# microsoft/SpeechT5

Hardware: AMD Instinct MI355X
Metric: audio-sec/s fwd+bwd SpeechT5-Base (higher is better)
Workload: dtype bf16

## Files before the change

### include/speecht5_hip.h

```cpp
#ifndef SPEECHT5_HIP_H
#define SPEECHT5_HIP_H
#include <stdint.h>
#ifdef __cplusplus
extern "C" {
#endif

#define ST5_F32 0
#define ST5_BF16 1

#define ST5_ACT_NONE 0
#define ST5_ACT_GELU 1
#define ST5_ACT_RELU 2
#define ST5_ACT_TANH 3
#define ST5_ACT_LRELU_01 4
#define ST5_ACT_LRELU_001 5

#define ST5_GEMM_A_KSTRIDED 1
#define ST5_GEMM_B_KSTRIDED 2
#define ST5_GEMM_OUT_F32 4
#define ST5_GEMM_DACT 8
#define ST5_GEMM_DEFERRABLE 16

typedef struct st5_operand {
  const void* ptr;
// ... 251 lines not shown
                     const int64_t* target_lengths, int32_t T, int32_t B, int32_t V, int32_t max_target_len, int32_t blank,
                     int32_t zero_infinity, const float* nll, const float* grad_out, const void* ws, float* grad, void* stream);
int64_t st5_guided_attn_ws_bytes(void);
int st5_guided_attn_fwd(const float* att, const int64_t* ilens, const int64_t* olens, int32_t B, int32_t H, int32_t To, int32_t Ti,
                        float sigma, float alpha, float* out2, void* ws, void* stream);
int st5_guided_attn_bwd(const int64_t* ilens, const int64_t* olens, int32_t B, int32_t H, int32_t To, int32_t Ti, float sigma,
                        const float* out2, const float* grad_out, float* datt, void* stream);
int64_t st5_vq_ws_bytes(void);
int32_t st5_vq_vpad(void);
int st5_vq_fwd(const float* logits, const float* gumbel, const float* vars, const void* enc, const float* mix_w, float tau, const float* tau_dev,
               int32_t training, void* out, int32_t* idx, float* avg, float* perp2, void* ws, int32_t N, int32_t G, int32_t V, int32_t Dg,
               int32_t T, int dtype, void* stream);
int st5_vq_bwd(const float* logits, const float* gumbel, const float* dsel, int32_t dsel_ld, const float* avg, const float* g_prob_perp,
               const void* dout, const float* mix_w, float tau, const float* tau_dev, int32_t training, float* dlogits, void* denc, int32_t N,
               int32_t G, int32_t V, int32_t Dg, int32_t T, int dtype, void* stream);
int st5_norm_rows(const void* x, float* y, float* inv, int64_t rows, int32_t cols, int dtype, void* stream);
int st5_norm_rows_bwd(const float* y, const float* inv, const float* dy, void* dx, int64_t rows, int32_t cols, int32_t accumulate, int dtype,
                      void* stream);
int st5_canon_rows(const float* e, int32_t* canon, int32_t V, int32_t D, void* stream);
int st5_nce_logits(const float* sim, const int32_t* target, const int32_t* canon, float* logits, int64_t S, int32_t V, float temp, void* stream);
int st5_nce_logits_bwd(const float* dlogits, const int32_t* target, const int32_t* canon, float* dsim, int32_t dsim_ld, int64_t S, int32_t V,
                       float temp, void* stream);
int st5_layernorm_set_max_blocks(int n);
int st5_ctc_initial_state(const float* x, int32_t T, int32_t V, int32_t blank, float* r, void* stream);
int st5_ctc_prefix_score(const float* x, int32_t T, int32_t V, int32_t blank, int32_t eos, const float* r_prev, const int64_t* last,
                         int32_t out_len, const int64_t* cs, int32_t nh, int32_t nc, float* log_psi, float* r_new, void* stream);
int st5_ctc_initial_state_rows(const float* x, const int32_t* lens, int32_t S, int32_t Tmax, int32_t V, int32_t blank, float* r, void* stream);
int st5_ctc_prefix_score_rows(const float* x, const int32_t* lens, const int32_t* sent, int32_t S, int32_t Tmax, int32_t V, int32_t blank,
                              int32_t eos, const float* r_prev, const int64_t* last, int32_t out_len, const int64_t* cs, int32_t nh,
                              int32_t nc, float* log_psi, float* r_new, void* stream);
int st5_ctc_select_rows(const int32_t* lens, const int32_t* sent, int32_t S, int32_t Tmax, const int64_t* cs, int32_t nh, int32_t nc,
                        const float* log_psi, const float* r_new, const int64_t* parent, const int64_t* token, int32_t n, float* state,
                        float* prev_psi, uint8_t* known, int32_t* sent_out, void* stream);
int64_t st5_lm_decode_attn_ws_bytes(int32_t rows, int32_t t, int32_t H, int32_t head_dim);
int st5_lm_decode_attn(const void* q, int64_t q_ld, const void* kv, int32_t rows_cap, int32_t Tmax, const int32_t* anc, int64_t anc_ld,
                       int32_t rows, int32_t t, int32_t H, int32_t head_dim, void* ctx, int64_t ctx_ld, float* ws, int dtype, void* stream);
int st5_lm_reorder(const int32_t* anc, int64_t anc_ld, const int64_t* order, int32_t rows_old, int32_t rows_new, int32_t t, int32_t Tmax,
                   int32_t* anc_new, int64_t new_ld, void* stream);
int st5_lm_fuse_logprobs(float* lprobs, int64_t lp_ld, const void* logits, int64_t lg_ld, int32_t rows, int32_t V_lm, float lm_weight,
                         int dtype, void* stream);
int64_t st5_decode_cross_attn_ws_bytes(int32_t B, int32_t S, int32_t H, int32_t head_dim);
int st5_decode_cross_attn(const void* q, int64_t q_ld, const void* kv, int64_t kv_ld, int64_t k_off, const uint8_t* kpm, int32_t B,
                          int32_t S, int32_t H, int32_t head_dim, void* ctx, int64_t ctx_ld, float* probs, int64_t p_row, int64_t p_head,
                          float* ws, int dtype, void* stream);
int st5_tts_step_tail(const float* y, int64_t y_ld, int32_t B, int32_t r, int32_t odim, const int32_t* minlen, const int32_t* maxlen,
                      int32_t* done, int32_t* steps, int32_t idx, int32_t cap, float threshold, float* mel, float* probs, void* next,
// ... 59 lines not shown
```

### speecht5_amd/csrc/norm.hip

```cpp
#include "common.h"
#include "../../include/speecht5_hip.h"

namespace {

constexpr int MAXCH = 8;

template <typename T, int NCH>
__device__ __forceinline__ void load_row(const T* row, int cols, int lane, bool vec, float (&v)[NCH][8]) {
#pragma unroll
  for (int i = 0; i < NCH; ++i) {
    const int c = i * 512 + lane * 8;
    if (c < cols) {
      if (vec) load8f<T>(row + c, v[i]);
      else {
#pragma unroll
        for (int e = 0; e < 8; ++e) v[i][e] = (c + e < cols) ? Elem<T>::to_f(row[c + e]) : 0.f;
      }
    } else {
#pragma unroll
      for (int e = 0; e < 8; ++e) v[i][e] = 0.f;
    }
  }
}
template <typename T, int NCH>
// ... 335 lines not shown
        const long long r2 = r1 + stride;
        if (r2 < rows) load_set(A, r2);
        finish_set(B, r1);
        if (r2 >= rows) break;
        row0 = r2;
      }
    }
  }
  if (PG) {
#pragma unroll
    for (int i = 0; i < NV; ++i) {
      const int c = (i * 64 + lane) * 4;
      if (c < cols) {
#pragma unroll
        for (int e = 0; e < 4; ++e) { red[(wave * 2 + 0) * cols + c + e] = dg[i][e]; red[(wave * 2 + 1) * cols + c + e] = db[i][e]; }
      }
    }
    __syncthreads();
    for (int c = threadIdx.x; c < 2 * cols; c += 256)
      part[(long long)blockIdx.x * 2 * cols + c] = red[c] + red[2 * cols + c] + red[4 * cols + c] + red[6 * cols + c];
  }
}

__global__ __launch_bounds__(1024) void ln_bwd_final_kernel(const float* __restrict__ part, float* __restrict__ dgamma,
                                                            float* __restrict__ dbeta, int nblk, int cols) {
  __shared__ float red[16][64];
  const int cl = threadIdx.x & 63, j = threadIdx.x >> 6;
  const int c = blockIdx.x * 64 + cl;
  float s = 0.f;
  if (c < 2 * cols)
    for (int b = j; b < nblk; b += 16) s += part[(long long)b * 2 * cols + c];
  red[j][cl] = s;
  __syncthreads();
  if (j == 0 && c < 2 * cols) {
    s = 0.f;
#pragma unroll
    for (int k = 0; k < 16; ++k) s += red[k][cl];
    if (c < cols) { if (dgamma) dgamma[c] += s; }
    else if (dbeta) dbeta[c - cols] += s;
  }
}

constexpr int LNF_MAX = 48;
struct LnFinalDesc { const float* part; float* dgamma; float* dbeta; int nblk, cols, blk0, pad; };
struct LnFinalArgs { LnFinalDesc d[LNF_MAX]; int n; };
__global__ __launch_bounds__(1024) void ln_bwd_final_multi_kernel(const LnFinalArgs a) {
// ... 29 lines not shown
    for (int i = 0; i < g_nlnstates; ++i)
      if (g_lnstates[i].pending.n != 0) return nullptr;
    if (hipDeviceSynchronize() != hipSuccess) return nullptr;
    g_nlnstates = 0;
  }
  LnDeferState* d = &g_lnstates[g_nlnstates++];
  d->stream = s; d->pending.n = 0; d->blocks = 0; d->arena_used = 0;
  return d;
}
#define g_ln_pending (ls->pending)
#define g_ln_blocks (ls->blocks)
#define g_ln_arena (ls->arena)
#define g_ln_arena_bytes (ls->arena_bytes)
#define g_ln_arena_used (ls->arena_used)
int ln_flush_state(LnDeferState* ls) {
  if (!ls || g_ln_pending.n == 0) return ST5_OK;
  hipLaunchKernelGGL(ln_bwd_final_multi_kernel, dim3((unsigned)g_ln_blocks), dim3(1024), 0, ls->stream, g_ln_pending);
  g_ln_pending.n = 0; g_ln_blocks = 0; g_ln_arena_used = 0;
  HIP_CHECK_LAUNCH();
  return ST5_OK;
}
int ln_flush(hipStream_t s) { return ln_flush_state(ln_state(s, false)); }

int ln_blocks(long long rows) {
  long long n = (rows + 4 * BRPW - 1) / (4 * BRPW);
  if (n < 1) n = 1;
  if (n <= g_ln_max_blocks) return (int)n;
  const long long trips = (n + g_ln_max_blocks - 1) / g_ln_max_blocks;
  return (int)((n + trips - 1) / trips);
}

template <typename T, int MODE>
__global__ __launch_bounds__(256) void colreduce_kernel(const T* __restrict__ x, const T* __restrict__ dy,
                                                        const float* __restrict__ mean,
                                                        const float* __restrict__ rstd, float* __restrict__ part,
                                                        long long rows, int cols, long long ld, const float* __restrict__ gate = nullptr) {
  if (st5_gate_dropped(gate)) return;
  __shared__ float red[8][256 + 8];
  const int tx = threadIdx.x & 31, ty = threadIdx.x >> 5;
  const int c0 = blockIdx.x * 256 + tx * 8;
  const bool vec = (ld % 8) == 0 && c0 + 8 <= cols;
  float acc[8];
#pragma unroll
  for (int e = 0; e < 8; ++e) acc[e] = 0.f;
  if (c0 < cols) {
    for (long long r = (long long)blockIdx.y * 8 + ty; r < rows; r += (long long)gridDim.y * 8) {
// ... 57 lines not shown
  dim3 grid((cols + 255) / 256, ns);
  hipLaunchKernelGGL((colreduce_kernel<T, MODE>), grid, dim3(256), 0, s, (const T*)x, (const T*)dy, mean, rstd, ws,
                     rows, cols, ld, gate);
  hipLaunchKernelGGL(colreduce_final_kernel, dim3((cols + 255) / 256), dim3(256), 0, s, ws, out, ns, cols, scale,
                     accumulate, gate);
  HIP_CHECK_LAUNCH();
  return ST5_OK;
}

}

static int layernorm_fwd(const void* x, const float* gamma, const float* beta, void* y, float* mean,
                         float* rstd, int64_t rows, int32_t cols, float eps, int dtype, void* stream, const float* keep, const void* skip,
                         const float* gate = nullptr) {
  if (!x || !y || !gamma || !beta || rows < 0 || cols <= 0 || cols > MAXCH * 512) return ST5_ERR_ARG;
  if (keep && (!skip || cols % 4 != 0 || cols > 2048)) return ST5_ERR_ARG;
  if (gate && ((skip && !keep) || cols % 4 != 0 || cols > 2048)) return ST5_ERR_ARG;
  if (rows == 0) return ST5_OK;
  hipStream_t s = (hipStream_t)stream;
  dim3 grid((unsigned)((rows + 3) / 4));
  if (dtype != ST5_BF16 && dtype != ST5_F32) return ST5_ERR_ARG;
  if (cols % 4 == 0 && cols <= 2048) {
    dim3 vgrid((unsigned)((rows + 4 * RPW - 1) / (4 * RPW)));
#define LNV(TT, NV_)                                                                                                 \
  hipLaunchKernelGGL((ln_fwd_vec_kernel<TT, NV_>), vgrid, dim3(256), 0, s, (const TT*)x, gamma, beta, (TT*)y, mean, rstd, \
                     (long long)rows, cols, eps, keep, (const TT*)skip, (unsigned char*)nullptr, (unsigned char*)nullptr, gate)
#define LNV_T(TT)                                                                                                     \
  do {                                                                                                                \
    if (cols <= 256) LNV(TT, 1); else if (cols <= 512) LNV(TT, 2); else if (cols <= 768) LNV(TT, 3);                  \
    else if (cols <= 1024) LNV(TT, 4); else if (cols <= 1536) LNV(TT, 6); else LNV(TT, 8);                            \
  } while (0)
    if (dtype == ST5_BF16) LNV_T(bf16_t); else LNV_T(float);
#undef LNV_T
#undef LNV
    HIP_CHECK_LAUNCH();
    return ST5_OK;
  }
#define LNF(TT, NCH)                                                                                              \
  hipLaunchKernelGGL((ln_fwd_kernel<TT, NCH>), grid, dim3(256), 0, s, (const TT*)x, gamma, beta, (TT*)y, mean, rstd, \
                     (long long)rows, cols, eps)
#define LNF_T(TT)                                                                                \
  do {                                                                                           \
    if (cols <= 512) LNF(TT, 1); else if (cols <= 1024) LNF(TT, 2); else if (cols <= 2048) LNF(TT, 4); else LNF(TT, 8); \
  } while (0)
  if (dtype == ST5_BF16) LNF_T(bf16_t); else LNF_T(float);
#undef LNF_T
#undef LNF
  HIP_CHECK_LAUNCH();
  return ST5_OK;
}

extern "C" int st5_layernorm_fwd(const void* x, const float* gamma, const float* beta, void* y, float* mean,
                                 float* rstd, int64_t rows, int32_t cols, float eps, int dtype, void* stream) {
  return layernorm_fwd(x, gamma, beta, y, mean, rstd, rows, cols, eps, dtype, stream, nullptr, nullptr);
}
extern "C" int st5_layernorm_fwd_q8(const void* x, const float* gamma, const float* beta, void* y, float* mean, float* rstd, void* q, uint8_t* sc,
                                    int64_t rows, int32_t cols, float eps, void* stream) {
  if (!x || !y || !gamma || !beta || !q || !sc || rows < 0 || cols <= 0 || cols % 32 || cols > 2048) return ST5_ERR_ARG;
  if (rows == 0) return ST5_OK;
  hipStream_t s = (hipStream_t)stream;
  dim3 vgrid((unsigned)((rows + 4 * RPW - 1) / (4 * RPW)));
#define LNQ(NV_)                                                                                                                       \
  hipLaunchKernelGGL((ln_fwd_vec_kernel<bf16_t, NV_, true>), vgrid, dim3(256), 0, s, (const bf16_t*)x, gamma, beta, (bf16_t*)y, mean, rstd, \
                     (long long)rows, cols, eps, (const float*)nullptr, (const bf16_t*)nullptr, (unsigned char*)q, (unsigned char*)sc)
  if (cols <= 256) LNQ(1); else if (cols <= 512) LNQ(2); else if (cols <= 768) LNQ(3);
  else if (cols <= 1024) LNQ(4); else if (cols <= 1536) LNQ(6); else LNQ(8);
#undef LNQ
  HIP_CHECK_LAUNCH();
  return ST5_OK;
}
extern "C" int st5_layernorm_gelu_fwd(const void* x, const float* gamma, const float* beta, void* y, float* mean, float* rstd,
                                      int64_t rows, int32_t cols, float eps, int dtype, void* stream) {
  if (!x || !y || !gamma || !beta || rows < 0 || cols <= 0 || cols % 4 || cols > 512) return ST5_ERR_ARG;
  if (dtype != ST5_BF16 && dtype != ST5_F32) return ST5_ERR_ARG;
  if (rows == 0) return ST5_OK;
  hipStream_t s = (hipStream_t)stream;
  dim3 vgrid((unsigned)((rows + 4 * RPW - 1) / (4 * RPW)));
#define LNA(TT, NV_)                                                                                                                      \
  hipLaunchKernelGGL((ln_fwd_vec_kernel<TT, NV_, false, true>), vgrid, dim3(256), 0, s, (const TT*)x, gamma, beta, (TT*)y, mean, rstd,    \
                     (long long)rows, cols, eps, (const float*)nullptr, (const TT*)nullptr, (unsigned char*)nullptr, (unsigned char*)nullptr)
  if (dtype == ST5_BF16) { if (cols <= 256) LNA(bf16_t, 1); else LNA(bf16_t, 2); }
  else { if (cols <= 256) LNA(float, 1); else LNA(float, 2); }
#undef LNA
  HIP_CHECK_LAUNCH();
  return ST5_OK;
}
extern "C" int st5_layernorm_gelu_bwd(const void* dy, const void* x, const float* gamma, const float* beta, const float* mean, const float* rstd,
                                      void* dx, float* dgamma, float* dbeta, void* ws, int64_t rows, int32_t cols, int dtype, void* stream) {
  if (!dy || !x || !gamma || !beta || !mean || !rstd || !dx || rows < 0 || cols <= 0 || cols % 4 || cols > 512) return ST5_ERR_ARG;
  if ((dgamma || dbeta) && !ws) return ST5_ERR_ARG;
  if (dtype != ST5_BF16 && dtype != ST5_F32) return ST5_ERR_ARG;
  if (rows == 0) return ST5_OK;
  hipStream_t s = (hipStream_t)stream;
  const int nb = ln_blocks(rows);
  const bool pg = dgamma || dbeta;
  const size_t shm = pg ? (size_t)8 * cols * sizeof(float) : 0;
#define LBA(TT, NV_)                                                                                                                       \
  do {                                                                                                                                     \
    if (pg) hipLaunchKernelGGL((ln_bwd_vec_kernel<TT, NV_, true, true>), dim3(nb), dim3(256), shm, s, (const TT*)dy, (const TT*)x, gamma,  \
                               mean, rstd, (TT*)dx, (float*)ws, (long long)rows, cols, (TT*)nullptr, 0.f, 0ull, (const float*)nullptr, beta); \
    else hipLaunchKernelGGL((ln_bwd_vec_kernel<TT, NV_, false, true>), dim3(nb), dim3(256), 0, s, (const TT*)dy, (const TT*)x, gamma,      \
                            mean, rstd, (TT*)dx, (float*)ws, (long long)rows, cols, (TT*)nullptr, 0.f, 0ull, (const float*)nullptr, beta); \
  } while (0)
  if (dtype == ST5_BF16) { if (cols <= 256) LBA(bf16_t, 1); else LBA(bf16_t, 2); }
  else { if (cols <= 256) LBA(float, 1); else LBA(float, 2); }
#undef LBA
  if (pg) hipLaunchKernelGGL(ln_bwd_final_kernel, dim3((2 * cols + 63) / 64), dim3(1024), 0, s, (const float*)ws, dgamma, dbeta, nb, cols);
  HIP_CHECK_LAUNCH();
  return ST5_OK;
}
extern "C" int st5_layernorm_gated_fwd(const void* x, const float* gamma, const float* beta, void* y, float* mean, float* rstd,
                                       int64_t rows, int32_t cols, float eps, const float* keep, const void* skip, int dtype, void* stream) {
  if (!keep || !skip) return ST5_ERR_ARG;
  return layernorm_fwd(x, gamma, beta, y, mean, rstd, rows, cols, eps, dtype, stream, keep, skip);
}
extern "C" int st5_layernorm_fwd_gate(const void* x, const float* gamma, const float* beta, void* y, float* mean, float* rstd, int64_t rows,
                                      int32_t cols, float eps, const float* keep, const void* skip, const float* gate, int dtype,
                                      void* stream) {
  if ((keep == nullptr) != (skip == nullptr)) return ST5_ERR_ARG;
  return layernorm_fwd(x, gamma, beta, y, mean, rstd, rows, cols, eps, dtype, stream, keep, skip, gate);
}

extern "C" int64_t st5_layernorm_bwd_ws_bytes(int64_t rows, int32_t cols) {
  const int64_t a = (int64_t)nsplit_for(rows) * cols * sizeof(float);
  const int64_t b = (int64_t)ln_blocks(rows) * 2 * cols * sizeof(float);
  return a > b ? a : b;
}

static int layernorm_bwd(const void* dy, const void* x, const float* gamma, const float* mean,
// ... 20 lines not shown
      for (int j = 0; j < g_ln_pending.n; ++j)
        if ((dgamma && g_ln_pending.d[j].dgamma == dgamma) || (dbeta && g_ln_pending.d[j].dbeta == dbeta)) {
          const int rc = ln_flush(s); if (rc) return rc; break;
        }
      const size_t need = ((size_t)nb * 2 * cols * sizeof(float) + 255) & ~(size_t)255;
      if (g_ln_pending.n == LNF_MAX || g_ln_arena_used + need > g_ln_arena_bytes) {
        const int rc = ln_flush(s); if (rc) return rc;
        if (need > g_ln_arena_bytes) {
          if (g_ln_arena) (void)hipFree(g_ln_arena);
          size_t want = size_t(128) << 20;
          while (want < need * 4) want *= 2;
          if (st5_dev_malloc(&g_ln_arena, want) != hipSuccess) { g_ln_arena = nullptr; g_ln_arena_bytes = 0; return ST5_ERR_LAUNCH; }
          g_ln_arena_bytes = want;
        }
      }
      ws = reinterpret_cast<char*>(g_ln_arena) + g_ln_arena_used;
      g_ln_arena_used += need;
      LnFinalDesc& d = g_ln_pending.d[g_ln_pending.n++];
      d.part = reinterpret_cast<const float*>(ws); d.dgamma = dgamma; d.dbeta = dbeta; d.nblk = nb; d.cols = cols;
      d.blk0 = g_ln_blocks; d.pad = 0;
      g_ln_blocks += (2 * cols + 63) / 64;
      deferred = true;
    }
#define LBV(TT, NV_)                                                                                                    \
  do {                                                                                                                  \
    if (pg) hipLaunchKernelGGL((ln_bwd_vec_kernel<TT, NV_, true>), dim3(nb), dim3(256), shm, s, (const TT*)dy, (const TT*)x, gamma, \
                               mean, rstd, (TT*)dx, (float*)ws, (long long)rows, cols, (TT*)dx_dropped, drop_p,          \
                               (unsigned long long)drop_seed, keep, (const float*)nullptr, (const TT*)addend, gate);    \
    else hipLaunchKernelGGL((ln_bwd_vec_kernel<TT, NV_, false>), dim3(nb), dim3(256), 0, s, (const TT*)dy, (const TT*)x, gamma, \
                            mean, rstd, (TT*)dx, (float*)ws, (long long)rows, cols, (TT*)dx_dropped, drop_p,            \
                            (unsigned long long)drop_seed, keep, (const float*)nullptr, (const TT*)addend, gate);       \
  } while (0)
#define LBV_T(TT)                                                                                                     \
  do {                                                                                                                \
    if (cols <= 256) LBV(TT, 1); else if (cols <= 512) LBV(TT, 2); else if (cols <= 768) LBV(TT, 3);                  \
    else if (cols <= 1024) LBV(TT, 4); else if (cols <= 1536) LBV(TT, 6); else LBV(TT, 8);                            \
  } while (0)
    if (dtype == ST5_BF16) LBV_T(bf16_t); else LBV_T(float);
#undef LBV_T
#undef LBV
    if (pg && !deferred) hipLaunchKernelGGL(ln_bwd_final_kernel, dim3((2 * cols + 63) / 64), dim3(1024), 0, s, (const float*)ws, dgamma, dbeta, nb, cols);
    HIP_CHECK_LAUNCH();
    return ST5_OK;
  }
  int rc = ST5_OK;
  if (dtype == ST5_BF16) {
    if (dgamma) rc |= colreduce<bf16_t, 1>(x, dy, mean, rstd, dgamma, (float*)ws, rows, cols, cols, 1.f, 1, s);
    if (dbeta) rc |= colreduce<bf16_t, 0>(dy, nullptr, nullptr, nullptr, dbeta, (float*)ws, rows, cols, cols, 1.f, 1, s);
  } else if (dtype == ST5_F32) {
    if (dgamma) rc |= colreduce<float, 1>(x, dy, mean, rstd, dgamma, (float*)ws, rows, cols, cols, 1.f, 1, s);
    if (dbeta) rc |= colreduce<float, 0>(dy, nullptr, nullptr, nullptr, dbeta, (float*)ws, rows, cols, cols, 1.f, 1, s);
  } else return ST5_ERR_ARG;
  if (rc) return rc;
  if (dx) {
    dim3 grid((unsigned)((rows + 3) / 4));
#define LNB(TT, NCH)                                                                                         \
  hipLaunchKernelGGL((ln_bwd_dx_kernel<TT, NCH>), grid, dim3(256), 0, s, (const TT*)dy, (const TT*)x, gamma, mean, \
                     rstd, (TT*)dx, (long long)rows, cols)
#define LNB_T(TT)                                                                                \
  do {                                                                                           \
    if (cols <= 512) LNB(TT, 1); else if (cols <= 1024) LNB(TT, 2); else if (cols <= 2048) LNB(TT, 4); else LNB(TT, 8); \
  } while (0)
    if (dtype == ST5_BF16) LNB_T(bf16_t); else LNB_T(float);
// ... 22 lines not shown
  return layernorm_bwd(dy, x, gamma, mean, rstd, dx, dgamma, dbeta, ws, rows, cols, dx_dropped, drop_p, drop_seed, dtype, stream, keep);
}
extern "C" int st5_layernorm_bwd_gate(const void* dy, const void* x, const float* gamma, const float* mean, const float* rstd, void* dx,
                                      float* dgamma, float* dbeta, void* ws, int64_t rows, int32_t cols, void* dx_dropped, float drop_p,
                                      uint64_t drop_seed, const float* keep, const float* gate, int dtype, void* stream) {
  return layernorm_bwd(dy, x, gamma, mean, rstd, dx, dgamma, dbeta, ws, rows, cols, dx_dropped, drop_p, drop_seed, dtype, stream, keep,
                       nullptr, gate);
}

#undef g_ln_pending
#undef g_ln_blocks
#undef g_ln_arena
#undef g_ln_arena_bytes
#undef g_ln_arena_used
extern "C" int st5_layernorm_defer(int enabled, void* stream) {
  (void)stream;
  if (!enabled && g_ln_defer) {
    for (int i = 0; i < g_nlnstates; ++i) { const int rc = ln_flush_state(&g_lnstates[i]); if (rc) return rc; }
  }
  g_ln_defer = enabled != 0;
  return ST5_OK;
}
extern "C" int st5_layernorm_flush(void* stream) { return ln_flush(reinterpret_cast<hipStream_t>(stream)); }
extern "C" int st5_layernorm_set_max_blocks(int n) { if (n < 1 || n > 4096) return ST5_ERR_ARG; g_ln_max_blocks = n; return ST5_OK; }

extern "C" int st5_colsum_ws(const void* x, float* out, void* ws, int64_t rows, int32_t cols, int64_t ld, float scale,
                             int32_t accumulate, int dtype, void* stream) {
  if (!x || !out || !ws || rows < 0 || cols <= 0) return ST5_ERR_ARG;
  hipStream_t s = (hipStream_t)stream;
  if (dtype == ST5_BF16)
    return colreduce<bf16_t, 0>(x, nullptr, nullptr, nullptr, out, (float*)ws, rows, cols, ld, scale, accumulate, s);
  if (dtype == ST5_F32)
    return colreduce<float, 0>(x, nullptr, nullptr, nullptr, out, (float*)ws, rows, cols, ld, scale, accumulate, s);
  return ST5_ERR_ARG;
}
extern "C" int st5_colsum_ws_gate(const void* x, float* out, void* ws, int64_t rows, int32_t cols, int64_t ld, float scale,
                                  int32_t accumulate, const float* gate, int dtype, void* stream) {
  if (!x || !out || !ws || rows < 0 || cols <= 0) return ST5_ERR_ARG;
  hipStream_t s = (hipStream_t)stream;
  if (dtype == ST5_BF16)
    return colreduce<bf16_t, 0>(x, nullptr, nullptr, nullptr, out, (float*)ws, rows, cols, ld, scale, accumulate, s, gate);
  if (dtype == ST5_F32)
    return colreduce<float, 0>(x, nullptr, nullptr, nullptr, out, (float*)ws, rows, cols, ld, scale, accumulate, s, gate);
  return ST5_ERR_ARG;
}
extern "C" int64_t st5_colsum_ws_bytes(int64_t rows, int32_t cols) {
// ... 3 lines not shown
```

### speecht5_amd/hip.py

```python
import ctypes
import os
from ctypes import POINTER, Structure, byref, c_char_p, c_float, c_int, c_int32, c_int64, c_uint64, c_void_p

import torch

F32, BF16 = 0, 1
ACT_NONE, ACT_GELU, ACT_RELU, ACT_TANH, ACT_LRELU_01, ACT_LRELU_001 = 0, 1, 2, 3, 4, 5
A_KSTRIDED, B_KSTRIDED, OUT_F32, DACT = 1, 2, 4, 8
DEFERRABLE = 16

_LIB_PATH = os.environ.get("ST5_HIP_LIB") or os.path.join(os.path.dirname(os.path.abspath(__file__)), "libspeecht5_hip.so")


class HipLibraryMissing(RuntimeError):
    pass


class HipKernelError(RuntimeError):
    pass


class Operand(Structure):
    _fields_ = [("ptr", c_void_p), ("ld", c_int64), ("rpb", c_int32), ("seg", c_int32),
                ("bstride", c_int64), ("seg_stride", c_int64), ("zs0", c_int64), ("zs1", c_int64)]
# ... 155 lines not shown
    "st5_ctc_loss_ws_bytes": (c_int64, [c_int32, c_int32, c_int32]),
    "st5_ctc_loss_fwd": (c_int, [c_void_p, c_void_p, c_void_p, c_void_p, c_void_p, c_int32, c_int32, c_int32, c_int32, c_int32, c_int32,
                                 c_void_p, c_void_p, c_void_p, c_void_p]),
    "st5_ctc_loss_bwd": (c_int, [c_void_p, c_void_p, c_void_p, c_void_p, c_void_p, c_int32, c_int32, c_int32, c_int32, c_int32, c_int32,
                                 c_void_p, c_void_p, c_void_p, c_void_p, c_void_p]),
    "st5_guided_attn_ws_bytes": (c_int64, []),
    "st5_guided_attn_fwd": (c_int, [c_void_p, c_void_p, c_void_p, c_int32, c_int32, c_int32, c_int32, c_float, c_float, c_void_p, c_void_p,
                                    c_void_p]),
    "st5_guided_attn_bwd": (c_int, [c_void_p, c_void_p, c_int32, c_int32, c_int32, c_int32, c_float, c_void_p, c_void_p, c_void_p, c_void_p]),
    "st5_vq_ws_bytes": (c_int64, []),
    "st5_vq_vpad": (c_int32, []),
    "st5_vq_fwd": (c_int, [c_void_p, c_void_p, c_void_p, c_void_p, c_void_p, c_float, c_void_p, c_int32, c_void_p, c_void_p, c_void_p, c_void_p,
                           c_void_p, c_int32, c_int32, c_int32, c_int32, c_int32, c_int, c_void_p]),
    "st5_vq_bwd": (c_int, [c_void_p, c_void_p, c_void_p, c_int32, c_void_p, c_void_p, c_void_p, c_void_p, c_float, c_void_p, c_int32, c_void_p,
                           c_void_p, c_int32, c_int32, c_int32, c_int32, c_int32, c_int, c_void_p]),
    "st5_norm_rows": (c_int, [c_void_p, c_void_p, c_void_p, c_int64, c_int32, c_int, c_void_p]),
    "st5_norm_rows_bwd": (c_int, [c_void_p, c_void_p, c_void_p, c_void_p, c_int64, c_int32, c_int32, c_int, c_void_p]),
    "st5_canon_rows": (c_int, [c_void_p, c_void_p, c_int32, c_int32, c_void_p]),
    "st5_nce_logits": (c_int, [c_void_p, c_void_p, c_void_p, c_void_p, c_int64, c_int32, c_float, c_void_p]),
    "st5_nce_logits_bwd": (c_int, [c_void_p, c_void_p, c_void_p, c_void_p, c_int32, c_int64, c_int32, c_float, c_void_p]),
    "st5_gather3": (c_int, [c_void_p, c_void_p, c_int32, c_int32, c_int32, c_int64, c_int64, c_int64, c_int64, c_int32, c_int, c_void_p]),
    "st5_zero_time_edges": (c_int, [c_void_p, c_int32, c_int32, c_int32, c_int32, c_int32, c_int, c_void_p]),
    "st5_layernorm_set_max_blocks": (c_int, [c_int]),
    "st5_adam_step_pair": (c_int, [c_void_p, c_void_p, c_void_p, c_int32, c_void_p, c_void_p, c_int64, c_float, c_float, c_float, c_float, c_float,
                                   c_int32, c_void_p, c_float, c_float, c_void_p, c_void_p, c_void_p]),
    "st5_sumsq_pair": (c_int, [c_void_p, c_void_p, c_void_p, c_int64, c_float, c_int32, c_void_p]),
    "st5_ctc_initial_state": (c_int, [c_void_p, c_int32, c_int32, c_int32, c_void_p, c_void_p]),
    "st5_ctc_prefix_score": (c_int, [c_void_p, c_int32, c_int32, c_int32, c_int32, c_void_p, c_void_p, c_int32, c_void_p, c_int32, c_int32,
                                     c_void_p, c_void_p, c_void_p]),
    "st5_ctc_initial_state_rows": (c_int, [c_void_p, c_void_p, c_int32, c_int32, c_int32, c_int32, c_void_p, c_void_p]),
    "st5_ctc_prefix_score_rows": (c_int, [c_void_p, c_void_p, c_void_p, c_int32, c_int32, c_int32, c_int32, c_int32, c_void_p, c_void_p,
                                          c_int32, c_void_p, c_int32, c_int32, c_void_p, c_void_p, c_void_p]),
    "st5_ctc_select_rows": (c_int, [c_void_p, c_void_p, c_int32, c_int32, c_void_p, c_int32, c_int32, c_void_p, c_void_p, c_void_p,
                                    c_void_p, c_int32, c_void_p, c_void_p, c_void_p, c_void_p, c_void_p]),
    "st5_lm_decode_attn_ws_bytes": (c_int64, [c_int32, c_int32, c_int32, c_int32]),
    "st5_lm_decode_attn": (c_int, [c_void_p, c_int64, c_void_p, c_int32, c_int32, c_void_p, c_int64, c_int32, c_int32, c_int32, c_int32,
                                   c_void_p, c_int64, c_void_p, c_int, c_void_p]),
    "st5_lm_reorder": (c_int, [c_void_p, c_int64, c_void_p, c_int32, c_int32, c_int32, c_int32, c_void_p, c_int64, c_void_p]),
    "st5_lm_fuse_logprobs": (c_int, [c_void_p, c_int64, c_void_p, c_int64, c_int32, c_int32, c_float, c_int, c_void_p]),
    "st5_decode_cross_attn_ws_bytes": (c_int64, [c_int32, c_int32, c_int32, c_int32]),
    "st5_decode_cross_attn": (c_int, [c_void_p, c_int64, c_void_p, c_int64, c_int64, c_void_p, c_int32, c_int32, c_int32, c_int32, c_void_p,
                                      c_int64, c_void_p, c_int64, c_int64, c_void_p, c_int, c_void_p]),
    "st5_tts_step_tail": (c_int, [c_void_p, c_int64, c_int32, c_int32, c_int32, c_void_p, c_void_p, c_void_p, c_void_p, c_int32, c_int32,
                                  c_float, c_void_p, c_void_p, c_void_p, c_int64, c_void_p, c_int, c_void_p]),
    "st5_gemm_skinny_ws_bytes": (c_int64, [c_int32, c_int32]),
    "st5_gemm_skinny": (c_int, [c_void_p, c_int64, c_void_p, c_int64, c_void_p, c_void_p, c_int64, c_void_p, c_int64, c_int32, c_int32, c_int32,
# ... 279 lines not shown
```

Measured before the change: 2960.

## Add streaming LayerNorm fwd/bwd kernels with software-pipelined row loads

Adds new LayerNorm forward and backward kernels that walk rows with a grid stride and issue raw vector loads for upcoming rows before finishing the current one. The forward kernel double-buffers rows, and the backward kernel keeps a small ring of in-flight rows sized by dtype and width. Both add a full-width specialization that uses immediate offsets. The goal is to hide memory latency in these bandwidth-bound kernels and to cap the forward grid. A runtime switch, on by default, selects the new path, while the keep-mask backward case still uses the old kernel. The extra in-flight registers may reduce occupancy.

```diff
diff --git a/include/speecht5_hip.h b/include/speecht5_hip.h
--- a/include/speecht5_hip.h
+++ b/include/speecht5_hip.h
@@ -297,6 +297,7 @@
 int st5_nce_logits_bwd(const float* dlogits, const int32_t* target, const int32_t* canon, float* dsim, int32_t dsim_ld, int64_t S, int32_t V,
                        float temp, void* stream);
 int st5_layernorm_set_max_blocks(int n);
+int st5_layernorm_set_impl(int impl);
 int st5_ctc_initial_state(const float* x, int32_t T, int32_t V, int32_t blank, float* r, void* stream);
 int st5_ctc_prefix_score(const float* x, int32_t T, int32_t V, int32_t blank, int32_t eos, const float* r_prev, const int64_t* last,
                          int32_t out_len, const int64_t* cs, int32_t nh, int32_t nc, float* log_psi, float* r_new, void* stream);
diff --git a/speecht5_amd/csrc/norm.hip b/speecht5_amd/csrc/norm.hip
--- a/speecht5_amd/csrc/norm.hip
+++ b/speecht5_amd/csrc/norm.hip
@@ -381,6 +381,307 @@
   }
 }
 
+int g_ln_impl = 1;
+constexpr int LN_FWD_MAX_BLOCKS = 1024;
+
+template <typename T> struct Raw4;
+template <> struct Raw4<float> { typedef f32x4 type; };
+template <> struct Raw4<bf16_t> { typedef u32x2 type; };
+__device__ __forceinline__ void raw_to_f(const f32x4& a, float (&v)[4]) {
+#pragma unroll
+  for (int i = 0; i < 4; ++i) v[i] = a[i];
+}
+__device__ __forceinline__ void raw_to_f(const u32x2& a, float (&v)[4]) {
+  v[0] = __uint_as_float(a[0] << 16); v[1] = __uint_as_float(a[0] & 0xffff0000u);
+  v[2] = __uint_as_float(a[1] << 16); v[3] = __uint_as_float(a[1] & 0xffff0000u);
+}
+template <typename T> __device__ __forceinline__ typename Raw4<T>::type f_to_raw(const float (&v)[4]);
+template <> __device__ __forceinline__ f32x4 f_to_raw<float>(const float (&v)[4]) {
+  f32x4 a;
+#pragma unroll
+  for (int i = 0; i < 4; ++i) a[i] = v[i];
+  return a;
+}
+template <> __device__ __forceinline__ u32x2 f_to_raw<bf16_t>(const float (&v)[4]) {
+  bf16x4 o;
+#pragma unroll
+  for (int i = 0; i < 4; ++i) o[i] = (bf16_t)v[i];
+  return __builtin_bit_cast(u32x2, o);
+}
+struct LaneOff { unsigned int v; int imm; };
+template <typename T> __device__ __forceinline__ typename Raw4<T>::type ld_raw(const T* row, const LaneOff off) {
+  unsigned int v = off.v;
+  asm volatile("" : "+v"(v));
+  return *reinterpret_cast<const typename Raw4<T>::type*>(reinterpret_cast<const char*>(row) + v + off.imm);
+}
+template <typename T> __device__ __forceinline__ void st_raw(T* row, const LaneOff off, const typename Raw4<T>::type& a) {
+  unsigned int v = off.v;
+  asm volatile("" : "+v"(v));
+  *reinterpret_cast<typename Raw4<T>::type*>(reinterpret_cast<char*>(row) + v + off.imm) = a;
+}
+template <typename T, int NV, bool FULL>
+__device__ __forceinline__ void lane_offsets(int lane, int cols, bool (&in)[NV], LaneOff (&off)[NV]) {
+#pragma unroll
+  for (int i = 0; i < NV; ++i) {
+    in[i] = FULL || (i * 64 + lane) * 4 < cols;
+    if (FULL) off[i] = LaneOff{(unsigned int)(lane * 4 * sizeof(T)), (int)(i * 256 * sizeof(T))};
+    else off[i] = LaneOff{in[i] ? (unsigned int)((i * 64 + lane) * 4 * sizeof(T)) : 0u, 0};
+  }
+}
+
+template <typename T, int NV, bool Q8, bool ACT, bool FULL>
+__global__ __launch_bounds__(256) void ln_fwd_stream_kernel(const T* __restrict__ x, const float* __restrict__ gamma,
+                                                            const float* __restrict__ beta, T* __restrict__ y,
+                                                            float* __restrict__ mean, float* __restrict__ rstd,
+                                                            long long rows, int cols, float eps,
+                                                            const float* __restrict__ keep, const T* __restrict__ skip,
+                                                            unsigned char* __restrict__ q8, unsigned char* __restrict__ s8,
+                                                            const float* __restrict__ gate) {
+#pragma clang fp contract(off)
+  typedef typename Raw4<T>::type Raw;
+  const int lane = threadIdx.x & 63;
+  const int wave = __builtin_amdgcn_readfirstlane((int)(threadIdx.x >> 6));
+  const long long stride = (long long)gridDim.x * 4;
+  long long row = (long long)blockIdx.x * 4 + wave;
+  bool in[NV];
+  LaneOff off[NV];
+  lane_offsets<T, NV, FULL>(lane, cols, in, off);
+  if (st5_gate_dropped(gate)) {
+    if (skip == nullptr) return;
+    for (; row < rows; row += stride) {
+      const long long ro = row * cols;
+#pragma unroll
+      for (int i = 0; i < NV; ++i)
+        if (in[i]) { float o[4]; raw_to_f(ld_raw<T>(skip + ro, off[i]), o); st_raw<T>(y + ro, off[i], f_to_raw<T>(o)); }
+    }
+    return;
+  }
+  const bool dropped = keep != nullptr && *keep == 0.f;
+  if (row >= rows) return;
+  float g[NV][4], b[NV][4];
+#pragma unroll
+  for (int i = 0; i < NV; ++i) {
+    const int c = (i * 64 + lane) * 4;
+    if (in[i]) { load4f<float>(gamma + c, g[i]); load4f<float>(beta + c, b[i]); }
+    else { g[i][0] = g[i][1] = g[i][2] = g[i][3] = 0.f; b[i][0] = b[i][1] = b[i][2] = b[i][3] = 0.f; }
+  }
+  const float inv_n = 1.f / (float)cols;
+  auto load_row = [&](Raw (&S)[NV], long long r) {
+    const T* const xr = x + r * cols;
+#pragma unroll
+    for (int i = 0; i < NV; ++i) S[i] = ld_raw<T>(xr, off[i]);
+  };
+  auto finish_row = [&](const Raw (&S)[NV], long long r) {
+    float v[NV][4];
+    float s = 0.f;
+#pragma unroll
+    for (int i = 0; i < NV; ++i) {
+      raw_to_f(S[i], v[i]);
+#pragma unroll
+      for (int e = 0; e < 4; ++e) { if (!FULL) v[i][e] = in[i] ? v[i][e] : 0.f; s += v[i][e]; }
+    }
+    const float tot = wave_sum(s);
+    const float mu = tot * inv_n;
+#pragma unroll
+    for (int i = 0; i < NV; ++i)
+#pragma unroll
+      for (int e = 0; e < 4; ++e) { const float d = fmaf(-inv_n, tot, v[i][e]); v[i][e] = (FULL || in[i]) ? d : 0.f; }
+    float q = fmaf(v[0][0], v[0][0], v[0][1] * v[0][1]);
+#pragma unroll
+    for (int i = 0; i < NV; ++i)
+#pragma unroll
+      for (int e = (i == 0 ? 2 : 0); e < 4; ++e) q = fmaf(v[i][e], v[i][e], q);
+    const float rs = rsqrtf(fmaf(wave_sum(q), inv_n, eps));
+    const long long ro = r * cols;
+#pragma unroll
+    for (int i = 0; i < NV; ++i) {
+      if (in[i]) {
+        float o[4];
+#pragma unroll
+        for (int e = 0; e < 4; ++e) o[e] = fmaf(v[i][e] * rs, g[i][e], b[i][e]);
+        if constexpr (ACT) {
+#pragma unroll
+          for (int e = 0; e < 4; ++e) o[e] = act_f<sizeof(T) == 2>(ACT_GELU, o[e]);
+        }
+        if (dropped) raw_to_f(ld_raw<T>(skip + ro, off[i]), o);
+        const Raw ob = f_to_raw<T>(o);
+        st_raw<T>(y + ro, off[i], ob);
+        if constexpr (Q8) {
+          const int c = (i * 64 + lane) * 4;
+          raw_to_f(ob, o);
+          unsigned int qw[1], qs;
+          mx8_quant<4>(o, qw, qs);
+          *reinterpret_cast<unsigned int*>(q8 + ro + c) = qw[0];
+          if ((lane & 7) == 0) s8[r * (cols >> 5) + (c >> 5)] = (unsigned char)qs;
+        }
+      }
+    }
+    if (lane == 0) { if (mean) mean[r] = mu; if (rstd) rstd[r] = rs; }
+  };
+  Raw A[NV], B[NV];
+  load_row(A, row);
+  while (true) {
+    const long long r1 = row + stride;
+    load_row(B, r1 < rows ? r1 : row);
+    finish_row(A, row);
+    if (r1 >= rows) break;
+    const long long r2 = r1 + stride;
+    load_row(A, r2 < rows ? r2 : r1);
+    finish_row(B, r1);
+    if (r2 >= rows) break;
+    row = r2;
+  }
+}
+
+template <typename T, int NV> constexpr int ln_ring() {
+  return 2 * NV * (int)sizeof(T) * 8 <= 128 ? 8 : (2 * NV * (int)sizeof(T) * 4 <= 128 ? 4 : 2);
+}
+
+template <typename T, int NV, bool PG, bool ACTB, bool FULL>
+__global__ __launch_bounds__(256) void ln_bwd_stream_kernel(const T* __restrict__ dy, const T* __restrict__ x,
+                                                            const float* __restrict__ gamma, const float* __restrict__ mean,
+                                                            const float* __restrict__ rstd, T* __restrict__ dx,
+                                                            float* __restrict__ part, long long rows, int cols,
+                                                            T* __restrict__ dxd, float drop_p, unsigned long long seed,
+                                                            const float* __restrict__ keep, const float* __restrict__ beta,
+                                                            const T* __restrict__ addend, const float* __restrict__ gate) {
+#pragma clang fp contract(off)
+  typedef typename Raw4<T>::type Raw;
+  constexpr int D = ln_ring<T, NV>();
+  (void)keep;
+  if (st5_gate_dropped(gate)) {
+    if (PG)
+      for (int c = threadIdx.x; c < 2 * cols; c += 256) part[(long long)blockIdx.x * 2 * cols + c] = 0.f;
+    return;
+  }
+  const unsigned int thresh = dxd ? dropout_thresh(drop_p) : 0u;
+  const float inv_keep = dxd ? 1.f / (1.f - drop_p) : 1.f;
+  const unsigned int seedf = dxd ? drop_seed_fold(seed) : 0u;
+  extern __shared__ float red[];
+  const int lane = threadIdx.x & 63;
+  const int wave = __builtin_amdgcn_readfirstlane((int)(threadIdx.x >> 6));
+  bool in[NV];
+  LaneOff off[NV];
+  lane_offsets<T, NV, FULL>(lane, cols, in, off);
+  float g[NV][4], dg[NV][4], db[NV][4];
+  float bb[ACTB ? NV : 1][4];
+#pragma unroll
+  for (int i = 0; i < NV; ++i) {
+    const int c = (i * 64 + lane) * 4;
+    if (in[i]) load4f<float>(gamma + c, g[i]);
+    else { g[i][0] = g[i][1] = g[i][2] = g[i][3] = 0.f; }
+    if constexpr (ACTB) {
+      if (in[i]) load4f<float>(beta + c, bb[i]);
+      else { bb[i][0] = bb[i][1] = bb[i][2] = bb[i][3] = 0.f; }
+    }
+#pragma unroll
+    for (int e = 0; e < 4; ++e) { dg[i][e] = 0.f; db[i][e] = 0.f; }
+  }
+  const float inv_n = 1.f / (float)cols;
+  const long long base = ((long long)blockIdx.x * 4 + wave) * BRPW;
+  const long long stride = (long long)gridDim.x * 4 * BRPW;
+  auto row_of = [&](long long j) {
+    const long long r = base + (j >> 2) * stride + (j & 3);
+    return (long long)(((unsigned long long)(unsigned int)__builtin_amdgcn_readfirstlane((int)(r >> 32)) << 32) |
+                       (unsigned int)__builtin_amdgcn_readfirstlane((int)r));
+  };
+  static_assert(BRPW == 4, "row_of");
+  auto issue = [&](Raw (&X)[NV], Raw (&G)[NV], float& m, float& r, long long row) {
+    const long long ro = row * cols;
+    const T* const xp = x + ro;
+    const T* const gp = dy + ro;
+#pragma unroll
+    for (int i = 0; i < NV; ++i) { X[i] = ld_raw<T>(xp, off[i]); G[i] = ld_raw<T>(gp, off[i]); }
+    m = mean[row]; r = rstd[row];
+  };
+  auto finish = [&](const Raw (&X)[NV], const Raw (&G)[NV], const float m, const float r, const long long row) {
+    float s1 = 0.f, s2 = 0.f;
+    float xh_[NV][4], gg_[NV][4];
+#pragma unroll
+    for (int i = 0; i < NV; ++i) {
+      float xv[4], dv[4];
+      raw_to_f(X[i], xv);
+      raw_to_f(G[i], dv);
+#pragma unroll
+      for (int e = 0; e < 4; ++e) {
+        float xh = (xv[e] - m) * r;
+        float d = dv[e];
+        if (!FULL) { xh = in[i] ? xh : 0.f; d = in[i] ? d : 0.f; }
+        if constexpr (ACTB) d *= act_grad_f<sizeof(T) == 2>(ACT_GELU, fmaf(xh, g[i][e], bb[i][e]));
+        if (PG) { dg[i][e] = fmaf(d, xh, dg[i][e]); db[i][e] += d; }
+        const float gg = d * g[i][e];
+        xh_[i][e] = xh; gg_[i][e] = gg;
+        s1 = fmaf(d, g[i][e], s1);
+        s2 = fmaf(gg, xh, s2);
+      }
+    }
+    const float s1t = wave_sum(s1);
+    s1 = s1t * inv_n;
+    s2 = wave_sum(s2) * inv_n;
+    const long long ro = row * cols;
+    T* const dxr = dx + ro;
+    const unsigned int t = ((unsigned int)ro & 63u) + (unsigned int)lane * 4u;
+    const unsigned int pc0 = ((t & 63u) >> 1) * 0x9E3779B1u, pc1 = pc0 + 0x9E3779B1u;
+    const unsigned long long bl = (unsigned long long)(ro >> 6) + (t >> 6);
+#pragma unroll
+    for (int i = 0; i < NV; ++i) {
+      if (in[i]) {
+        float o[4];
+#pragma unroll
+        for (int e = 0; e < 4; ++e)
+          o[e] = r * fmaf(-xh_[i][e], s2, NV == 1 ? fmaf(-inv_n, s1t, gg_[i][e]) : gg_[i][e] - s1);
+        if (addend) {
+          float a4[4];
+          raw_to_f(ld_raw<T>(addend + ro, off[i]), a4);
+#pragma unroll
+          for (int e = 0; e < 4; ++e) o[e] += a4[e];
+        }
+        const Raw ob = f_to_raw<T>(o);
+        st_raw<T>(dxr, off[i], ob);
+        if (dxd) {
+          T* const dr = dxd + ro;
+          const unsigned int key = drop_block_key_folded(seedf, bl + 4u * i);
+          const unsigned int b0 = drop_pair_bits_pc(key, pc0), b1 = drop_pair_bits_pc(key, pc1);
+          raw_to_f(ob, o);
+          o[0] *= drop_pick(b0, 0, thresh, inv_keep); o[1] *= drop_pick(b0, 1, thresh, inv_keep);
+          o[2] *= drop_pick(b1, 0, thresh, inv_keep); o[3] *= drop_pick(b1, 1, thresh, inv_keep);
+          st_raw<T>(dr, off[i], f_to_raw<T>(o));
+        }
+      }
+    }
+  };
+  if (base < rows) {
+    for (long long j0 = 0; row_of(j0) < rows; j0 += D) {
+      Raw xr[D][NV], gr[D][NV];
+      float mu[D], rs[D];
+#pragma unroll
+      for (int s = 0; s < D; ++s) {
+        const long long r = row_of(j0 + s);
+        issue(xr[s], gr[s], mu[s], rs[s], r < rows ? r : base);
+      }
+#pragma unroll
+      for (int s = 0; s < D; ++s) {
+        const long long row = row_of(j0 + s);
+        if (row >= rows) break;
+        finish(xr[s], gr[s], mu[s], rs[s], row);
+      }
+    }
+  }
+  if (PG) {
+#pragma unroll
+    for (int i = 0; i < NV; ++i) {
+      const int c = (i * 64 + lane) * 4;
+      if (in[i]) {
+#pragma unroll
+        for (int e = 0; e < 4; ++e) { red[(wave * 2 + 0) * cols + c + e] = dg[i][e]; red[(wave * 2 + 1) * cols + c + e] = db[i][e]; }
+      }
+    }
+    __syncthreads();
+    for (int c = threadIdx.x; c < 2 * cols; c += 256)
+      part[(long long)blockIdx.x * 2 * cols + c] = red[c] + red[2 * cols + c] + red[4 * cols + c] + red[6 * cols + c];
+  }
+}
+
 __global__ __launch_bounds__(1024) void ln_bwd_final_kernel(const float* __restrict__ part, float* __restrict__ dgamma,
                                                             float* __restrict__ dbeta, int nblk, int cols) {
   __shared__ float red[16][64];
@@ -456,6 +757,11 @@
 }
 int ln_flush(hipStream_t s) { return ln_flush_state(ln_state(s, false)); }
 
+dim3 ln_fwd_stream_grid(long long rows) {
+  const long long n = (rows + 3) / 4;
+  return dim3((unsigned)(n < LN_FWD_MAX_BLOCKS ? n : LN_FWD_MAX_BLOCKS));
+}
+
 int ln_blocks(long long rows) {
   long long n = (rows + 4 * BRPW - 1) / (4 * BRPW);
   if (n < 1) n = 1;
@@ -559,9 +865,15 @@
   if (dtype != ST5_BF16 && dtype != ST5_F32) return ST5_ERR_ARG;
   if (cols % 4 == 0 && cols <= 2048) {
     dim3 vgrid((unsigned)((rows + 4 * RPW - 1) / (4 * RPW)));
+    const dim3 sgrid = ln_fwd_stream_grid(rows);
+#define LNV_ARGS(TT) (const TT*)x, gamma, beta, (TT*)y, mean, rstd, (long long)rows, cols, eps, keep, (const TT*)skip,  \
+                     (unsigned char*)nullptr, (unsigned char*)nullptr, gate
 #define LNV(TT, NV_)                                                                                                 \
-  hipLaunchKernelGGL((ln_fwd_vec_kernel<TT, NV_>), vgrid, dim3(256), 0, s, (const TT*)x, gamma, beta, (TT*)y, mean, rstd, \
-                     (long long)rows, cols, eps, keep, (const TT*)skip, (unsigned char*)nullptr, (unsigned char*)nullptr, gate)
+  do {                                                                                                               \
+    if (g_ln_impl == 0) hipLaunchKernelGGL((ln_fwd_vec_kernel<TT, NV_>), vgrid, dim3(256), 0, s, LNV_ARGS(TT));      \
+    else if (cols == NV_ * 256) hipLaunchKernelGGL((ln_fwd_stream_kernel<TT, NV_, false, false, true>), sgrid, dim3(256), 0, s, LNV_ARGS(TT)); \
+    else hipLaunchKernelGGL((ln_fwd_stream_kernel<TT, NV_, false, false, false>), sgrid, dim3(256), 0, s, LNV_ARGS(TT)); \
+  } while (0)
 #define LNV_T(TT)                                                                                                     \
   do {                                                                                                                \
     if (cols <= 256) LNV(TT, 1); else if (cols <= 512) LNV(TT, 2); else if (cols <= 768) LNV(TT, 3);                  \
@@ -570,6 +882,7 @@
     if (dtype == ST5_BF16) LNV_T(bf16_t); else LNV_T(float);
 #undef LNV_T
 #undef LNV
+#undef LNV_ARGS
     HIP_CHECK_LAUNCH();
     return ST5_OK;
   }
@@ -597,12 +910,19 @@
   if (rows == 0) return ST5_OK;
   hipStream_t s = (hipStream_t)stream;
   dim3 vgrid((unsigned)((rows + 4 * RPW - 1) / (4 * RPW)));
+  const dim3 sgrid = ln_fwd_stream_grid(rows);
+#define LNQ_ARGS (const bf16_t*)x, gamma, beta, (bf16_t*)y, mean, rstd, (long long)rows, cols, eps, (const float*)nullptr,              \
+                 (const bf16_t*)nullptr, (unsigned char*)q, (unsigned char*)sc, (const float*)nullptr
 #define LNQ(NV_)                                                                                                                       \
-  hipLaunchKernelGGL((ln_fwd_vec_kernel<bf16_t, NV_, true>), vgrid, dim3(256), 0, s, (const bf16_t*)x, gamma, beta, (bf16_t*)y, mean, rstd, \
-                     (long long)rows, cols, eps, (const float*)nullptr, (const bf16_t*)nullptr, (unsigned char*)q, (unsigned char*)sc)
+  do {                                                                                                                                 \
+    if (g_ln_impl == 0) hipLaunchKernelGGL((ln_fwd_vec_kernel<bf16_t, NV_, true>), vgrid, dim3(256), 0, s, LNQ_ARGS);                  \
+    else if (cols == NV_ * 256) hipLaunchKernelGGL((ln_fwd_stream_kernel<bf16_t, NV_, true, false, true>), sgrid, dim3(256), 0, s, LNQ_ARGS); \
+    else hipLaunchKernelGGL((ln_fwd_stream_kernel<bf16_t, NV_, true, false, false>), sgrid, dim3(256), 0, s, LNQ_ARGS);               \
+  } while (0)
   if (cols <= 256) LNQ(1); else if (cols <= 512) LNQ(2); else if (cols <= 768) LNQ(3);
   else if (cols <= 1024) LNQ(4); else if (cols <= 1536) LNQ(6); else LNQ(8);
 #undef LNQ
+#undef LNQ_ARGS
   HIP_CHECK_LAUNCH();
   return ST5_OK;
 }
@@ -613,12 +933,19 @@
   if (rows == 0) return ST5_OK;
   hipStream_t s = (hipStream_t)stream;
   dim3 vgrid((unsigned)((rows + 4 * RPW - 1) / (4 * RPW)));
+  const dim3 sgrid = ln_fwd_stream_grid(rows);
+#define LNA_ARGS(TT) (const TT*)x, gamma, beta, (TT*)y, mean, rstd, (long long)rows, cols, eps, (const float*)nullptr, (const TT*)nullptr, \
+                     (unsigned char*)nullptr, (unsigned char*)nullptr, (const float*)nullptr
 #define LNA(TT, NV_)                                                                                                                      \
-  hipLaunchKernelGGL((ln_fwd_vec_kernel<TT, NV_, false, true>), vgrid, dim3(256), 0, s, (const TT*)x, gamma, beta, (TT*)y, mean, rstd,    \
-                     (long long)rows, cols, eps, (const float*)nullptr, (const TT*)nullptr, (unsigned char*)nullptr, (unsigned char*)nullptr)
+  do {                                                                                                                                    \
+    if (g_ln_impl == 0) hipLaunchKernelGGL((ln_fwd_vec_kernel<TT, NV_, false, true>), vgrid, dim3(256), 0, s, LNA_ARGS(TT));              \
+    else if (cols == NV_ * 256) hipLaunchKernelGGL((ln_fwd_stream_kernel<TT, NV_, false, true, true>), sgrid, dim3(256), 0, s, LNA_ARGS(TT)); \
+    else hipLaunchKernelGGL((ln_fwd_stream_kernel<TT, NV_, false, true, false>), sgrid, dim3(256), 0, s, LNA_ARGS(TT));                   \
+  } while (0)
   if (dtype == ST5_BF16) { if (cols <= 256) LNA(bf16_t, 1); else LNA(bf16_t, 2); }
   else { if (cols <= 256) LNA(float, 1); else LNA(float, 2); }
 #undef LNA
+#undef LNA_ARGS
   HIP_CHECK_LAUNCH();
   return ST5_OK;
 }
@@ -632,16 +959,22 @@
   const int nb = ln_blocks(rows);
   const bool pg = dgamma || dbeta;
   const size_t shm = pg ? (size_t)8 * cols * sizeof(float) : 0;
+#define LBA_ARGS(TT) (const TT*)dy, (const TT*)x, gamma, mean, rstd, (TT*)dx, (float*)ws, (long long)rows, cols, (TT*)nullptr, 0.f, 0ull,   \
+                     (const float*)nullptr, beta, (const TT*)nullptr, (const float*)nullptr
+#define LBA_K(TT, NV_, PG_)                                                                                                                \
+  do {                                                                                                                                     \
+    if (g_ln_impl == 0) hipLaunchKernelGGL((ln_bwd_vec_kernel<TT, NV_, PG_, true>), dim3(nb), dim3(256), PG_ ? shm : 0, s, LBA_ARGS(TT));  \
+    else if (cols == NV_ * 256)                                                                                                            \
+      hipLaunchKernelGGL((ln_bwd_stream_kernel<TT, NV_, PG_, true, true>), dim3(nb), dim3(256), PG_ ? shm : 0, s, LBA_ARGS(TT));           \
+    else hipLaunchKernelGGL((ln_bwd_stream_kernel<TT, NV_, PG_, true, false>), dim3(nb), dim3(256), PG_ ? shm : 0, s, LBA_ARGS(TT));       \
+  } while (0)
 #define LBA(TT, NV_)                                                                                                                       \
-  do {                                                                                                                                     \
-    if (pg) hipLaunchKernelGGL((ln_bwd_vec_kernel<TT, NV_, true, true>), dim3(nb), dim3(256), shm, s, (const TT*)dy, (const TT*)x, gamma,  \
-                               mean, rstd, (TT*)dx, (float*)ws, (long long)rows, cols, (TT*)nullptr, 0.f, 0ull, (const float*)nullptr, beta); \
-    else hipLaunchKernelGGL((ln_bwd_vec_kernel<TT, NV_, false, true>), dim3(nb), dim3(256), 0, s, (const TT*)dy, (const TT*)x, gamma,      \
-                            mean, rstd, (TT*)dx, (float*)ws, (long long)rows, cols, (TT*)nullptr, 0.f, 0ull, (const float*)nullptr, beta); \
-  } while (0)
+  do { if (pg) LBA_K(TT, NV_, true); else LBA_K(TT, NV_, false); } while (0)
   if (dtype == ST5_BF16) { if (cols <= 256) LBA(bf16_t, 1); else LBA(bf16_t, 2); }
   else { if (cols <= 256) LBA(float, 1); else LBA(float, 2); }
 #undef LBA
+#undef LBA_K
+#undef LBA_ARGS
   if (pg) hipLaunchKernelGGL(ln_bwd_final_kernel, dim3((2 * cols + 63) / 64), dim3(1024), 0, s, (const float*)ws, dgamma, dbeta, nb, cols);
   HIP_CHECK_LAUNCH();
   return ST5_OK;
@@ -708,15 +1041,17 @@
       g_ln_blocks += (2 * cols + 63) / 64;
       deferred = true;
     }
+#define LBV_ARGS(TT) (const TT*)dy, (const TT*)x, gamma, mean, rstd, (TT*)dx, (float*)ws, (long long)rows, cols, (TT*)dx_dropped, drop_p, \
+                     (unsigned long long)drop_seed, keep, (const float*)nullptr, (const TT*)addend, gate
+#define LBV_K(TT, NV_, PG_)                                                                                             \
+  do {                                                                                                                  \
+    if (g_ln_impl == 0 || keep) hipLaunchKernelGGL((ln_bwd_vec_kernel<TT, NV_, PG_>), dim3(nb), dim3(256), PG_ ? shm : 0, s, LBV_ARGS(TT)); \
+    else if (cols == NV_ * 256)                                                                                         \
+      hipLaunchKernelGGL((ln_bwd_stream_kernel<TT, NV_, PG_, false, true>), dim3(nb), dim3(256), PG_ ? shm : 0, s, LBV_ARGS(TT)); \
+    else hipLaunchKernelGGL((ln_bwd_stream_kernel<TT, NV_, PG_, false, false>), dim3(nb), dim3(256), PG_ ? shm : 0, s, LBV_ARGS(TT)); \
+  } while (0)
 #define LBV(TT, NV_)                                                                                                    \
-  do {                                                                                                                  \
-    if (pg) hipLaunchKernelGGL((ln_bwd_vec_kernel<TT, NV_, true>), dim3(nb), dim3(256), shm, s, (const TT*)dy, (const TT*)x, gamma, \
-                               mean, rstd, (TT*)dx, (float*)ws, (long long)rows, cols, (TT*)dx_dropped, drop_p,          \
-                               (unsigned long long)drop_seed, keep, (const float*)nullptr, (const TT*)addend, gate);    \
-    else hipLaunchKernelGGL((ln_bwd_vec_kernel<TT, NV_, false>), dim3(nb), dim3(256), 0, s, (const TT*)dy, (const TT*)x, gamma, \
-                            mean, rstd, (TT*)dx, (float*)ws, (long long)rows, cols, (TT*)dx_dropped, drop_p,            \
-                            (unsigned long long)drop_seed, keep, (const float*)nullptr, (const TT*)addend, gate);       \
-  } while (0)
+  do { if (pg) LBV_K(TT, NV_, true); else LBV_K(TT, NV_, false); } while (0)
 #define LBV_T(TT)                                                                                                     \
   do {                                                                                                                \
     if (cols <= 256) LBV(TT, 1); else if (cols <= 512) LBV(TT, 2); else if (cols <= 768) LBV(TT, 3);                  \
@@ -725,6 +1060,8 @@
     if (dtype == ST5_BF16) LBV_T(bf16_t); else LBV_T(float);
 #undef LBV_T
 #undef LBV
+#undef LBV_K
+#undef LBV_ARGS
     if (pg && !deferred) hipLaunchKernelGGL(ln_bwd_final_kernel, dim3((2 * cols + 63) / 64), dim3(1024), 0, s, (const float*)ws, dgamma, dbeta, nb, cols);
     HIP_CHECK_LAUNCH();
     return ST5_OK;
@@ -793,6 +1130,7 @@
   return ST5_OK;
 }
 extern "C" int st5_layernorm_flush(void* stream) { return ln_flush(reinterpret_cast<hipStream_t>(stream)); }
+extern "C" int st5_layernorm_set_impl(int impl) { if (impl != 0 && impl != 1) return ST5_ERR_ARG; g_ln_impl = impl; return ST5_OK; }
 extern "C" int st5_layernorm_set_max_blocks(int n) { if (n < 1 || n > 4096) return ST5_ERR_ARG; g_ln_max_blocks = n; return ST5_OK; }
 
 extern "C" int st5_colsum_ws(const void* x, float* out, void* ws, int64_t rows, int32_t cols, int64_t ld, float scale,
diff --git a/speecht5_amd/hip.py b/speecht5_amd/hip.py
--- a/speecht5_amd/hip.py
+++ b/speecht5_amd/hip.py
@@ -201,6 +201,7 @@
     "st5_gather3": (c_int, [c_void_p, c_void_p, c_int32, c_int32, c_int32, c_int64, c_int64, c_int64, c_int64, c_int32, c_int, c_void_p]),
     "st5_zero_time_edges": (c_int, [c_void_p, c_int32, c_int32, c_int32, c_int32, c_int32, c_int, c_void_p]),
     "st5_layernorm_set_max_blocks": (c_int, [c_int]),
+    "st5_layernorm_set_impl": (c_int, [c_int]),
     "st5_adam_step_pair": (c_int, [c_void_p, c_void_p, c_void_p, c_int32, c_void_p, c_void_p, c_int64, c_float, c_float, c_float, c_float, c_float,
                                    c_int32, c_void_p, c_float, c_float, c_void_p, c_void_p, c_void_p]),
     "st5_sumsq_pair": (c_int, [c_void_p, c_void_p, c_void_p, c_int64, c_float, c_int32, c_void_p]),
```

Result: no change. 2983 (median of 6 runs) (+0.8%).
